# Sangluisme/PSgradientSDF

Hardware: AMD Instinct MI355X
Metric: Gauss-Newton iterations/sec (full PS sweep), 256^3 grid x 50 frames (higher is better)
Workload: dtype f32

## Files before the change

### psgradientsdf_amd/capi.py

```python
from __future__ import annotations

import ctypes as C
import os

import numpy as np

ALBEDO, LIGHT, DIST, POSE, ALL = 1, 2, 4, 8, 15
SH1, SH2, LED = 0, 1, 2
L2, CAUCHY, HUBER, TUKEY, TRUNC_L2 = 0, 1, 2, 3, 4
R_DEPTH, R_NORMAL, R_ALBEDO, R_SHADING, R_RENDERED, R_RESIDUAL, R_VOXEL = 1, 2, 4, 8, 16, 32, 64
R_ALL = 127
_R_PLANES = [("depth", R_DEPTH, 1), ("normal", R_NORMAL, 3), ("albedo", R_ALBEDO, 3), ("shading", R_SHADING, 1),
             ("rendered", R_RENDERED, 3), ("residual", R_RESIDUAL, 3), ("voxel", R_VOXEL, 1)]

_HERE = os.path.dirname(os.path.abspath(__file__))
ENGINE_LIB = os.environ.get("PSGSDF_ENGINE_LIB") or os.path.join(_HERE, "csrc", "libpsgsdf.so")
ENGINE_LIB_DEV = os.path.join(_HERE, "csrc", "libpsgsdf_dev.so")


class GridDesc(C.Structure):
    _fields_ = [("dim", C.c_int32 * 3), ("voxel_size", C.c_float), ("shift", C.c_float * 3), ("truncation", C.c_float)]


class Settings(C.Structure):
# ... 439 lines not shown
    def watch_kernel(self, name):
        self._check(self._fn("watch_kernel")(self.ctx, name.encode() if name else None), "watch_kernel")

    def reset_kernel_times(self):
        self._check(self._fn("reset_kernel_times")(self.ctx), "reset_kernel_times")

    def kernel_times(self):
        cap = 64
        names = (C.c_char_p * cap)(); ms = (C.c_double * cap)(); n = (C.c_int64 * cap)()
        f = getattr(self._lib, self._p + "kernel_times"); f.restype = C.c_int
        k = f(self.ctx, names, ms, n, C.c_int(cap))
        return {names[i].decode(): (ms[i], n[i]) for i in range(k)}

    def debug_dist_system(self, x=None):
        S = self.info().n_band
        diag = np.empty(S, np.float32); rhs = np.empty(S, np.float32)
        y = np.empty(S, np.float32) if x is not None else None
        xa = np.ascontiguousarray(x, np.float32) if x is not None else None
        self._check(self._fn("debug_dist_system")(self.ctx, diag.ctypes.data_as(C.c_void_p), rhs.ctypes.data_as(C.c_void_p),
                                                   xa.ctypes.data_as(C.c_void_p) if x is not None else None,
                                                   y.ctypes.data_as(C.c_void_p) if x is not None else None), "debug_dist_system")
        return diag, rhs, y

    def debug_time_pcg_pass(self, blocks=0, rows=2, ablate=0, reps=50, stamps=False):
        ms = C.c_double(0)
        st = np.zeros((max(blocks, 1), 8), np.int64) if stamps else None
        self._check(self._fn("debug_time_pcg_pass")(self.ctx, C.c_int(blocks), C.c_int(rows), C.c_int(ablate | (1024 if stamps else 0)), C.c_int(reps), C.byref(ms),
                                                     st.ctypes.data_as(C.c_void_p) if stamps else None), "debug_time_pcg_pass")
        return (ms.value, st) if stamps else ms.value

    def debug_time_pcg_solve(self, passes=16, reps=5):
        ms = C.c_double(0); shape = (C.c_int32 * 2)(); st = (C.c_double * 16)()
        self._check(self._fn("debug_time_pcg_solve")(self.ctx, C.c_int(passes), C.c_int(reps), C.byref(ms), shape, st), "debug_time_pcg_solve")
        return ms.value, (shape[0], shape[1]), [x for x in st]

    def debug_sync_stats(self):
        out = (C.c_int64 * 8)()
        self._check(self._fn("debug_sync_stats")(self.ctx, out), "debug_sync_stats")
        return dict(readbacks_checked=out[0], readbacks_late=out[1], persist_fallbacks=out[2] % 1000000, keyframes_compacted=out[2] // 1000000, speculative_starts=out[3] // 1000000, speculative_undos=out[3] % 1000000,
                    cross_rank_ready=out[4] % 10, halo_pushes=out[4] // 10, cross_rank_solves=out[5], cross_rank_mem_kind=out[6], probe_stale=out[7] // 1000000, probe_timeouts=out[7] % 1000000)

    def debug_rare_rows(self):
        r = C.c_int64(); w = C.c_int64()
        self._check(self._fn("debug_rare_rows")(self.ctx, C.byref(r), C.byref(w)), "debug_rare_rows")
        return r.value, w.value

# ... 79 lines not shown
```

### psgradientsdf_amd/csrc/api_debug.hip

```cpp
#include "engine_internal.h"

using namespace psge;

extern "C" {
int psgsdf_set_profiling(psgsdf_ctx* c, int enabled) { if (!c) return PSGSDF_ERR_ARG; c->profiling = enabled != 0; return PSGSDF_OK; }
int psgsdf_reset_kernel_times(psgsdf_ctx* c) { if (!c) return PSGSDF_ERR_ARG; c->ktimes.clear(); c->watch_used = 0; return PSGSDF_OK; }
int psgsdf_watch_kernel(psgsdf_ctx* c, const char* name) {
    if (!c) return PSGSDF_ERR_ARG;
    hipStreamSynchronize(c->stream);
    std::string w = name ? name : ""; int every = 1;
    const size_t sl = w.find('/');
    if (sl != std::string::npos) { every = std::max(1, atoi(w.c_str() + sl + 1)); w.resize(sl); }
    c->watch = w; c->watch_every = every; c->watch_seen = 0; c->watch_used = 0;
    return PSGSDF_OK;
}
int psgsdf_kernel_times(psgsdf_ctx* c, const char** names, double* ms, int64_t* launches, int cap) {
    if (!c) return 0;
    if (c->watch_used) {
        hipStreamSynchronize(c->stream);
        KTime& k = c->ktimes[c->watch];
        for (size_t i = 0; i < c->watch_used; ++i) { float t = 0; if (hipEventElapsedTime(&t, c->watch_pool[i].first, c->watch_pool[i].second) == hipSuccess) { k.ms += t; k.n += 1; } }
        c->watch_used = 0;
    }
    int n = 0;
    for (auto& kv : c->ktimes) { if (n >= cap) break; names[n] = kv.first.c_str(); ms[n] = kv.second.ms; launches[n] = kv.second.n; ++n; }
    return n;
}

int psgsdf_debug_dist_system(psgsdf_ctx* c, float* diag, float* rhs, const float* x, float* y) {
    if (!c || !c->inited) return fail(c, PSGSDF_ERR_STATE, "init first");
    HIPCHK(c, hipSetDevice(c->device));
    SweepArgs a = make_args(c, c->reg_l != 0.f);
    launch_sweep_dist(a, c->stream);
    launch_assemble(a, c->stream);
    const int S = c->band.S;
    if (diag) HIPCHK(c, hipMemcpyAsync(diag, c->band.H, sizeof(float) * S, hipMemcpyDeviceToHost, c->stream));
    if (rhs) HIPCHK(c, hipMemcpyAsync(rhs, c->band.rhs, sizeof(float) * S, hipMemcpyDeviceToHost, c->stream));
    if (x && y) {
        HIPCHK(c, hipMemcpyAsync(c->band.x, x, sizeof(float) * S, hipMemcpyHostToDevice, c->stream));
        launch_matvec(a, c->band.x, c->band.t, c->stream);
        HIPCHK(c, hipMemcpyAsync(y, c->band.t, sizeof(float) * S, hipMemcpyDeviceToHost, c->stream));
    }
    HIPCHK(c, hipStreamSynchronize(c->stream));
    return PSGSDF_OK;
}

int psgsdf_debug_time_pcg_pass(psgsdf_ctx* c, int blocks, int rows, int ablate, int reps, double* avg_ms, long long* stamps) {
    if (!c || !c->inited || !avg_ms) return fail(c, PSGSDF_ERR_STATE, "init first");
    HIPCHK(c, hipSetDevice(c->device));
    SweepArgs a = make_args(c, c->reg_l != 0.f);
    launch_sweep_dist(a, c->stream);
    launch_assemble(a, c->stream);
    int G, rdef; cgf_shape(band_blocks(c), &G, &rdef);
    if (blocks > 0) G = std::min(blocks, kCgfMaxBlocks);
    if (rows <= 0) rows = rdef;
    launch_cgf_init(a, c->pcg_sc, c->pcg_part, G, c->stream);
    hipEvent_t e0, e1; HIPCHK(c, hipEventCreate(&e0)); HIPCHK(c, hipEventCreate(&e1));
    for (int q = 0; q < 3; ++q) launch_cgf_pass(a, c->pcg_sc, c->pcg_part, G, rows, q, 1 << 30, c->mbox_dev, c->stream, ablate | 16);
    HIPCHK(c, hipEventRecord(e0, c->stream));
    for (int q = 0; q < reps; ++q) launch_cgf_pass(a, c->pcg_sc, c->pcg_part, G, rows, 3 + q, 1 << 30, c->mbox_dev, c->stream, ablate | 16);
    HIPCHK(c, hipEventRecord(e1, c->stream));
    HIPCHK(c, hipStreamSynchronize(c->stream));
    float ms = 0; HIPCHK(c, hipEventElapsedTime(&ms, e0, e1));
    hipEventDestroy(e0); hipEventDestroy(e1);
    *avg_ms = (double)ms / reps;
    if (stamps) {
// ... 216 lines not shown
```

### psgradientsdf_amd/csrc/band.hip

```cpp
#include "device_common.h"

namespace psg {


__global__ void __launch_bounds__(kBlock) k_select_vis(const uint64_t* __restrict__ vis_seq, int wpv_seq, uint64_t* __restrict__ vis_key, int KW, const int* __restrict__ frame_idx, int F, long long nvox) {
    for (long long lin = blockIdx.x * (long long)blockDim.x + threadIdx.x; lin < nvox; lin += (long long)gridDim.x * blockDim.x) {
        if (wpv_seq <= 2) {
            const uint64_t s0 = vis_seq[lin * wpv_seq], s1 = wpv_seq > 1 ? vis_seq[lin * wpv_seq + 1] : 0ull;
            for (int w = 0; w < KW; ++w) {
                uint64_t out = 0;
                if (s0 | s1) {
                    const int f1 = min(F, 64 * (w + 1));
                    for (int f = 64 * w; f < f1; ++f) {
                        const int s = frame_idx[f];
                        const uint64_t word = s < 64 ? s0 : s1;
                        if (s >= 0 && s < 64 * wpv_seq && ((word >> (s & 63)) & 1ull)) out |= 1ull << (f & 63);
                    }
                }
                vis_key[lin * KW + w] = out;
            }
            continue;
        }
        for (int w = 0; w < KW; ++w) {
            uint64_t out = 0;
// ... 109 lines not shown
        if (!(q & 1) && r >= 0) fwd |= 1 << (q >> 1);
    }
    b.dirb[j] = fwd;
    int dl[kNQ], far = 0;
    for (int q = 0; q < kNQ; ++q) {
        int o[3]; q_offset(q, o);
        long long ln = lin + o[0] * stride[0] + o[1] * stride[1] + o[2] * stride[2];
        int r = (ln >= 0 && ln < grid.nvox) ? d.row_of[ln] : -1;
        b.col[(size_t)q * b.Spad + j] = r >= 0 ? r : j;
        dl[q] = r >= 0 ? r - j : 0;
        far = max(far, abs(dl[q]));
    }
    for (int w = 0; w < (kNQ - 1) / 2; ++w)
        b.colp[(size_t)w * b.Spad + j] = ((unsigned)dl[2 * w + 1] & 0xffffu) | ((unsigned)dl[2 * w + 2] << 16);
#pragma unroll
    for (int o = 32; o > 0; o >>= 1) far = max(far, __shfl_down(far, o, 64));
    if ((threadIdx.x & 63) == 0 && far > 0) atomicMax(reach, far);
}
void launch_band_fill(const DenseView& d, const GridP& grid, Band b, int* d_reach, hipStream_t s) {
    int g1 = (int)min((grid.nvox + kBlock - 1) / kBlock, (long long)256 * 16);
    hipLaunchKernelGGL(k_band_fill, dim3(g1), dim3(kBlock), 0, s, d, grid, b);
    if (b.S > 0) hipLaunchKernelGGL(k_band_nb, dim3((b.S + kBlock - 1) / kBlock), dim3(kBlock), 0, s, d, grid, b, d_reach);
}
__global__ void __launch_bounds__(kBlock) k_band_scatter(DenseView d, Band b) {
    int j = blockIdx.x * blockDim.x + threadIdx.x;
    if (j >= b.S) return;
    long long lin = b.lin[j];
    d.dist[lin] = b.dist[j];
#pragma unroll
    for (int a = 0; a < 3; ++a) { d.g[a][lin] = b.g[a][j]; d.rho[a][lin] = b.rho[a][j]; }
}
void launch_band_scatter(const DenseView& d, Band b, hipStream_t s) {
    if (b.S > 0) hipLaunchKernelGGL(k_band_scatter, dim3((b.S + kBlock - 1) / kBlock), dim3(kBlock), 0, s, d, b);
}

__global__ void __launch_bounds__(kBlock) k_upsample(DenseView src, DenseView dst, GridP g) {
    const long long nx = 2LL * g.dim[0], ny = 2LL * g.dim[1], nn = 8 * g.nvox;
    const float vs4 = (float)(0.25 * (double)g.vs);
    for (long long ls = blockIdx.x * (long long)blockDim.x + threadIdx.x; ls < nn; ls += (long long)gridDim.x * blockDim.x) {
        long long kz = ls / (nx * ny); long long rest = ls - kz * nx * ny; long long jy = rest / nx; long long ix = rest - jy * nx;
        long long lin = (ix >> 1) + (jy >> 1) * g.dim[0] + (kz >> 1) * (long long)g.dim[0] * g.dim[1];
        float d = src.dist[lin];
        if (d == g.T) {
            dst.dist[ls] = g.T; dst.weight[ls] = 0.f;
#pragma unroll
            for (int a = 0; a < 3; ++a) { dst.g[a][ls] = 0.f; dst.rho[a][ls] = 0.5f; }
// ... 148 lines not shown
```

### psgradientsdf_amd/csrc/device_common.h

```cpp
#pragma once
#include "engine.h"
#include <float.h>

#ifndef PSG_STRICT
#define PSG_STRICT 0
#endif
#if PSG_STRICT & 1
#pragma clang fp contract(off)
#else
#pragma clang fp contract(fast)
#endif

namespace psg {
#if PSG_STRICT & 8
typedef double obs_acc_t;
#else
typedef float obs_acc_t;
#endif

typedef float f2_t __attribute__((ext_vector_type(2)));
__device__ __forceinline__ float dot3(const float* a, const float* b) { return (a[0] * b[0] + a[1] * b[1]) + a[2] * b[2]; }
__device__ __forceinline__ float norm3(const float* a) { return sqrtf(dot3(a, a)); }
__device__ __forceinline__ void normalized3(const float* v, float* o) {
#pragma clang fp contract(off)
// ... 629 lines not shown
    float e = norm3(n) - 1; en = (double)(e * e);
    float l = laplacian(b, j, a.grid.vs_inv); el = (double)(l * l);
}

#define FOR_EACH_VISIBLE_FRAME(b, j, F, f)                                                   \
    for (int _w = 0; _w < (b).KW; ++_w)                                                      \
        for (uint64_t _m = (b).vis[(size_t)_w * (b).Spad + (j)]; _m; _m &= _m - 1)            \
            if (int f = 64 * _w + __builtin_ctzll(_m); f < (F))

struct PiRows { float p00, p02, p11, p12; };
__device__ __forceinline__ PiRows pi_rows(const Cam& cam, const Proj& pr) {
    const float z_inv = pr.z_inv, z_inv_sq = z_inv * z_inv;
    PiRows o; o.p00 = cam.fx * z_inv; o.p02 = -cam.fx * pr.p[0] * z_inv_sq; o.p11 = cam.fy * z_inv; o.p12 = -cam.fy * pr.p[1] * z_inv_sq;
    return o;
}
__device__ __forceinline__ void pi_rows_world(const PiRows& pi, const float* R, float* U, float* V) {
#pragma unroll
    for (int k = 0; k < 3; ++k) { U[k] = pi.p00 * R[k * 3 + 0] + pi.p02 * R[k * 3 + 2]; V[k] = pi.p11 * R[k * 3 + 1] + pi.p12 * R[k * 3 + 2]; }
}
__device__ __forceinline__ int sym4(int a, int b) {
    if (a > b) { int t = a; a = b; b = t; }
    return a * 4 - (a * (a - 1)) / 2 + (b - a);
}

__device__ inline void so3_exp(const float* w, float* R) {
    float theta_sq = dot3(w, w);
    float imag, real;
    if (theta_sq < 1e-10f) {
        float theta_po4 = theta_sq * theta_sq;
        imag = 0.5f - (1.0f / 48.0f) * theta_sq + (1.0f / 3840.0f) * theta_po4;
        real = 1.0f - (1.0f / 8.0f) * theta_sq + (1.0f / 384.0f) * theta_po4;
    } else {
        float theta = sqrtf(theta_sq), half = 0.5f * theta;
        imag = sinf(half) / theta; real = cosf(half);
    }
    float qw = real, qx = imag * w[0], qy = imag * w[1], qz = imag * w[2];
    float tx = 2 * qx, ty = 2 * qy, tz = 2 * qz;
    float twx = tx * qw, twy = ty * qw, twz = tz * qw, txx = tx * qx, txy = ty * qx, txz = tz * qx, tyy = ty * qy, tyz = tz * qy, tzz = tz * qz;
    R[0] = 1 - (tyy + tzz); R[1] = txy - twz; R[2] = txz + twy;
    R[3] = txy + twz; R[4] = 1 - (txx + tzz); R[5] = tyz - twx;
    R[6] = txz - twy; R[7] = tyz + twx; R[8] = 1 - (txx + tyy);
}
__device__ inline void pose_update(FrameP* frames, int f, const float* xi) {
    float R[9], t[3];
    for (int i = 0; i < 9; ++i) R[i] = frames[f].R[i];
    for (int i = 0; i < 3; ++i) t[i] = frames[f].t[i];
// ... 10 lines not shown
```

### psgradientsdf_amd/csrc/dist.hip

```cpp
#include "device_common.h"

#ifndef PSG_DIST_PK
#define PSG_DIST_PK 1
#endif

namespace psg {

__device__ __forceinline__ void normal_jacobian(float vs_inv, const float* grad, const float* direction, float* J) {
    float n_d[3] = {-vs_inv * direction[0], -vs_inv * direction[1], -vs_inv * direction[2]};
    float N_inv = (float)(1.0 / (double)fmaxf(norm3(grad), 0.001f));
    double Nd = (double)N_inv;
    float dN = (float)((Nd * Nd * Nd) * (double)dot3(n_d, grad));
#pragma unroll
    for (int k = 0; k < 3; ++k) J[k] = N_inv * n_d[k] - dN * grad[k];
}

template <int MODEL, int LOSS, int IMG>
__global__ void __launch_bounds__(kBlock, 4) k_sweep_dist(SweepArgs a) {
    constexpr int NB = ModelTraits<MODEL>::NB;
    constexpr bool LED = ModelTraits<MODEL>::LED;
    FrameP* sf = reinterpret_cast<FrameP*>(psg_dyn_smem);
    __shared__ double red[kBlock / 64];
    load_frames(sf, a.frames, a.F);
    const Band& b = a.b;
// ... 215 lines not shown
            float n_d[3] = {-vs_inv * dir[0], -vs_inv * dir[1], -vs_inv * dir[2]};
            float Jr[4];
            Jr[0] = dot3(grad, n_d);
#pragma unroll
            for (int k = 0; k < 3; ++k) Jr[k + 1] = grad[k] * (vs_inv * dir[k]);
            float gnrm = norm3(grad);
            if (gnrm > 0.0f) {
#pragma unroll
                for (int k = 0; k < 4; ++k) Jr[k] /= gnrm;
            }
            float res = gnrm - 1;
            int q = 0;
#pragma unroll
            for (int p = 0; p < 4; ++p) {
#pragma unroll
                for (int k = p; k < 4; ++k) B[q++] += (obs_acc_t)(a.reg_n * (Jr[p] * Jr[k]));
                g[p] += (obs_acc_t)(a.reg_n * (Jr[p] * res));
            }
        }
        if (a.laplacian_reg) {
            float vs2 = vs_inv * vs_inv; float Jl = -6 * vs2; float res = laplacian(b, j, vs_inv);
            B[0] += (obs_acc_t)(a.reg_l * (Jl * Jl)); g[0] += (obs_acc_t)(a.reg_l * (Jl * res));
        }
        int q = 0;
#pragma unroll
        for (int p = 0; p < 4; ++p) {
#pragma unroll
            for (int k = p; k < 4; ++k) { b.blk[(size_t)q * b.Spad + j] = (exists[p] && exists[k]) ? (float)B[q] : 0.f; ++q; }
        }
#pragma unroll
        for (int p = 0; p < 4; ++p) b.blk[(size_t)(10 + p) * b.Spad + j] = exists[p] ? (float)g[p] : 0.f;
    }
    block_part_store(E, PART(a, SC_ENERGY), red, bid);
    block_part_store(nobs, PART(a, SC_NOBS), red, bid);
    if (a.pcg_asm && a.pcg_gran) {
        if (blockIdx.x == 0 && threadIdx.x == 0) { a.pcg_fs[1] = 0.0; a.pcg_fs[2] = 0.0; a.pcg_fs[3] = 0.0; }
        const int gid = blockIdx.x * blockDim.x + threadIdx.x;
        for (int q = gid; q < a.pcg_gran_n; q += gridDim.x * blockDim.x) a.pcg_gran[q] = 0.0;
    }
}
void launch_sweep_dist(const SweepArgs& a, hipStream_t s) {
    if (a.row1 <= a.row0) return;
    dim3 g((a.row1 - a.row0 + kBlock - 1) / kBlock), bl(kBlock);
    PSG_LAUNCH_SWEEP(k_sweep_dist, a, false, g, bl, a.F * sizeof(FrameP), s, a);
}

__device__ __forceinline__ double assemble_row(const SweepArgs& a, int i, double (*acc)[kBlock]) {
    const Band& b = a.b;
    const int tid = threadIdx.x;
    double bb = 0.0;
    int jr[7]; jr[0] = i;
#pragma unroll
    for (int c = 1; c < 7; ++c) { const int ax = (c - 1) >> 1; const bool upper = (c - 1) & 1; jr[c] = b.nb[(size_t)(2 * ax + (upper ? 0 : 1)) * b.Spad + i]; }
    int db[7];
#pragma unroll
    for (int c = 0; c < 7; ++c) db[c] = b.dirb[jr[c] >= 0 ? jr[c] : i];
    bool use[7]; use[0] = true;
#pragma unroll
    for (int c = 1; c < 7; ++c) { const int ax = (c - 1) >> 1; const bool upper = (c - 1) & 1; use[c] = jr[c] >= 0 && !(upper && ((db[c] >> ax) & 1)); }
    float val[7][4], gr[7];
#pragma unroll
    for (int c = 0; c < 7; ++c) {
        const int s = c == 0 ? 0 : ((c - 1) >> 1) + 1;
        const int jrow = use[c] ? jr[c] : i;
        gr[c] = b.blk[(size_t)(10 + s) * b.Spad + jrow];
#pragma unroll
        for (int bq = 0; bq < 4; ++bq) val[c][bq] = b.blk[(size_t)sym4(s, bq) * b.Spad + jrow];
    }
    double rhs = 0.0;
#pragma unroll
    for (int c = 0; c < 7; ++c) {
        if (!use[c]) continue;
        const int ax = c == 0 ? 0 : (c - 1) >> 1; const bool upper = c > 0 && ((c - 1) & 1);
        int coff[3] = {0, 0, 0};
        if (c > 0) coff[ax] = upper ? 1 : -1;
        rhs += (double)gr[c];
#pragma unroll
        for (int bq = 0; bq < 4; ++bq) {
            int o[3] = {coff[0], coff[1], coff[2]};
            if (bq > 0) o[bq - 1] += ((db[c] >> (bq - 1)) & 1) ? 1 : -1;
            if (val[c][bq] != 0.f) acc[q_of(o)][tid] += (double)val[c][bq];
        }
    }
    int extra = 0;
#pragma unroll
    for (int q = 0; q < kNQ; ++q) { float h = (float)acc[q][tid]; b.H[(size_t)q * b.Spad + i] = h; if (q >= kNQCommon && h != 0.f) extra = 1; }
    b.hx[i] = extra;
    b.rhs[i] = (float)rhs;
    if (a.pcg_fuse_init) {
        float dg = (float)acc[0][tid];
        if (a.damping != 0.0f) dg += a.damping * dg;
// ... 32 lines not shown
```

### psgradientsdf_amd/csrc/engine.h

```cpp
#pragma once
#include <hip/hip_runtime.h>
#include <stdint.h>

namespace psg {

constexpr int kBlock = 256;
constexpr int kMaxFramesLds = 640;
constexpr int kNQ = 19;
constexpr int kNQCommon = 13;
constexpr int kMaxBasis = 9;

struct FrameP {
    float R[9];
    float t[3];
    float l[9];
    float pad[3];
};

struct Cam { float fx, fy, cx, cy; int W, H; };

struct GridP {
    int dim[3];
    long long nvox;
    float vs, vs_inv;
// ... 1 lines not shown
    float T;
    int koff;
};

struct Robust { int loss; float lambda, lambda_sq, inv_lambda; };

struct Band {
    int S, Spad, KW;
    int* lin;
    float* dist;
    float* g[3];
    float* rho[3];
    uint64_t* vis;
    int* nb;
    int* dirb;
    float* nbd;
    int* col;
    unsigned* colp;
    int col16;
    int reach;
    float* gfd[3];
    float4* vp[3];
    float* aH; float* ab;
    float* blk;
    float* H;
    int* hx;
    float* rhs; float* x; float* t;
    float4* rec[2];
    int* obs_ptr;
    int* obs_rows;
    int obs_max;
    long long obs_ptr_total;
};

struct Accum {
    double* frame;
    double* part;
    int PB;
    double* fpart;
    int fcap;
    int* fdone;
};
constexpr int kFrameRow = 64;
constexpr int kPcgMaxBlocks = 2048;
constexpr int kCgfMaxBlocks = 768;

enum { SC_ENERGY = 0, SC_NOBS = 1, SC_EN = 2, SC_EL = 3, SC_ACCEPT = 4, SC_AUX0 = 5, SC_AUX1 = 6, SC_AUX2 = 7, SC_COUNT = 8 };
// ... 57 lines not shown
};

constexpr int kXrMaxRanks = 32;
constexpr int kXrPeerTags = 64;
constexpr int kXrRankGran = 0, kXrPtag = 2 * 8 * kXrMaxRanks, kXrAbort = kXrPtag + 2 * 3 * kXrPeerTags, kXrDoubles = kXrAbort + 8;
constexpr int kXrLate = kXrAbort + 1;
constexpr int kXrNonce = kXrAbort + 7;
struct XrArgs {
    int rank, n_ranks;
    double* region[kXrMaxRanks];
    float4* lo_rec[2]; float4* hi_rec[2];
    float4* lo_base[2];
    int give_lo, give_hi;
    int wait_lo, wait_hi;
    int need_lo, need_hi;
    unsigned epoch;
};
struct XfTable {
    int n_ranks, rank, F, spin_max;
    long long pay, flg;
    long long spay, sflg;
    double* region[32];
};
constexpr int kHxWords = 16;
constexpr unsigned kXrEpochMask = 0x3fffu;

constexpr int kTryPackFlags = 2048;
void launch_normals_cache(int W, int H, int r, double fx_inv, double fy_inv, double cx, double cy, double* work , float* out , hipStream_t s);
void launch_try_pack_f32(const float* rgb, unsigned* rgba, size_t npix, size_t stride, float scale, int* fail , hipStream_t s);
void launch_pack_rgb8(const uint8_t* rgb, unsigned* rgba, size_t npix, hipStream_t s);
void launch_select_vis(const uint64_t* vis_seq, int wpv_seq, uint64_t* vis_key, int KW, const int* frame_idx, int F, long long nvox, hipStream_t s);
void launch_band_flags(const float* dist, const uint64_t* vis_key, int KW, float vs, long long nvox, int* flags, hipStream_t s);
void launch_band_scan(int* flags_inout_rowof, long long nvox, int* block_sums, int* d_total, hipStream_t s);
struct DenseView { float* dist; float* g[3]; float* weight; float* rho[3]; uint64_t* vis; int KW; int* row_of; };
void launch_band_fill(const DenseView& d, const GridP& grid, Band b, int* d_reach, hipStream_t s);
void launch_band_scatter(const DenseView& d, Band b, hipStream_t s);
void launch_derive(const SweepArgs& a, int update_grad, hipStream_t s);
constexpr int kObsChunk = 2048;
void launch_obs_count(const Band& b, int F, int row0, int row1, int* counts, hipStream_t s);
void launch_block_work(const Band& b, int row0, int row1, int* work, hipStream_t s);
void launch_obs_fill(const Band& b, int F, int row0, int row1, const int* offsets, hipStream_t s);
void launch_lower_bound(const int* lin, int S, int target, int* out, hipStream_t s);
struct SlotList { int n; int id[8]; };
void launch_sum_parts(const double* part, int PB, int nblk, const SlotList& slots, double* out, unsigned long long key, hipStream_t s, const XfTable* xf = nullptr, long long xf_epoch = 0);
void launch_frame_cols(const double* frame, int F, int col, double* out, unsigned long long key, hipStream_t s);
void launch_zero_f64(double* p, int n, hipStream_t s);
struct CopySegs { int n; unsigned off[16]; unsigned len[16]; unsigned long long key[16]; };
void launch_copy_segs(const double* src, double* dst, const CopySegs& segs, hipStream_t s);
void launch_marker(double* p, double v, hipStream_t s);
void launch_init_albedo(const SweepArgs& a, hipStream_t s);
void launch_led_light_init(const SweepArgs& a, hipStream_t s);
void launch_energy(const SweepArgs& a, hipStream_t s);
void launch_sweep_albedo(const SweepArgs& a, hipStream_t s);
void launch_apply_albedo(const SweepArgs& a, hipStream_t s);
void launch_restore_albedo(const SweepArgs& a, hipStream_t s);
int launch_sweep_light(const SweepArgs& a, hipStream_t s);
int launch_sweep_pose(const SweepArgs& a, hipStream_t s);
void launch_solve_light(const SweepArgs& a, FrameP* frames, float* led_light, double* e_out, unsigned long long e_key, float* undo, hipStream_t s);
// ... 92 lines not shown
```

### psgradientsdf_amd/csrc/engine.hip

```cpp
#include "engine_internal.h"
#include <chrono>
#include <sched.h>

namespace psge {

int wait_mapped(psgsdf_ctx* c, const std::function<bool()>& ready, const char* what) {
    using clk = std::chrono::steady_clock;
    static const double limit_s = [] { const char* e = getenv("PSGSDF_WAIT_TIMEOUT_S"); double v = e ? atof(e) : 0.0; return v > 0.0 ? v : 120.0; }();
    clk::time_point t0{}, next_query{};
    bool timing = false;
    for (unsigned spin = 1;; ++spin) {
        if (ready()) return 0;
        if (spin & 0x3ffu) continue;
        const clk::time_point now = clk::now();
        if (!timing) { timing = true; t0 = now; next_query = now + std::chrono::milliseconds(20); continue; }
        if (now - t0 > std::chrono::milliseconds(2)) sched_yield();
        if (now < next_query) continue;
        next_query = now + std::chrono::milliseconds(20);
        const hipError_t q = hipStreamQuery(c->stream);
        if (q == hipSuccess) return ready() ? 0 : 1;
        if (q != hipErrorNotReady) return fail(c, PSGSDF_ERR_DEVICE, "%s: stream error while waiting: %s", what, hipGetErrorString(q));
        if (std::chrono::duration<double>(now - t0).count() > limit_s)
            return fail(c, PSGSDF_ERR_DEVICE, "%s: nothing published within %.0f s (PSGSDF_WAIT_TIMEOUT_S)", what, limit_s);
    }
// ... 193 lines not shown
    HIPCHK(c, hipMalloc(&d.dist, sizeof(float) * nvox));
    for (int a = 0; a < 3; ++a) { HIPCHK(c, hipMalloc(&d.g[a], sizeof(float) * nvox)); HIPCHK(c, hipMalloc(&d.rho[a], sizeof(float) * nvox)); }
    HIPCHK(c, hipMalloc(&d.weight, sizeof(float) * nvox));
    d.KW = KW;
    if (KW > 0) HIPCHK(c, hipMalloc(&d.vis, sizeof(uint64_t) * nvox * KW));
    if (with_rowof) HIPCHK(c, hipMalloc(&d.row_of, sizeof(int) * nvox));
    return 0;
}

int build_band(psgsdf_ctx* c) {
    if (!c->deferred.empty() || c->pending_fold.n) { int rc = flush(c); if (rc) return rc; }
    if (xr_quiesce(c, 120.0)) return fail(c, PSGSDF_ERR_COMM, "band rebuild: a rank never closed its mappings of this rank's record planes (lost or failed peer?)");
    if (c->n_ranks > 1 && c->comm) { int rc = xr_probe(c); if (rc) return rc; }
    c->persist_off = false;
    const long long nvox = c->grid.nvox;
    const int KW = c->dense.KW;
    if (!c->block_sums) HIPCHK(c, hipMalloc(&c->block_sums, sizeof(int) * ((nvox + 1023) / 1024 + 1)));
    timed(c, "band_flags", [&] { launch_band_flags(c->dense.dist, c->dense.vis, KW, c->grid.vs, nvox, c->dense.row_of, c->stream); });
    timed(c, "band_scan", [&] { launch_band_scan(c->dense.row_of, nvox, c->block_sums, c->d_total, c->stream); });
    int S = 0;
    HIPCHK(c, hipMemcpyAsync(&S, c->d_total, sizeof(int), hipMemcpyDeviceToHost, c->stream));
    HIPCHK(c, hipStreamSynchronize(c->stream));
    const int Spad = ((S + kBlock - 1) / kBlock) * kBlock + kBlock;
    const size_t n4 = 1 + 1 + 3 + 3 + 6 + 6 + kNQ + 12 + 6 + 14 + kNQ + 4 + 9 + 1 + 3;
    const size_t bytes = (n4 * 4 + (size_t)KW * 8) * Spad + 256;
    if (c->band_mem) { hipFree(c->band_mem); c->band_mem = nullptr; }
    if (c->rec_mem) { hipFree(c->rec_mem); c->rec_mem = nullptr; }
    HIPCHK(c, hipMalloc(&c->band_mem, bytes));
    HIPCHK(c, hipMemsetAsync(c->band_mem, 0, bytes, c->stream));
    { int rc = xr_alloc(c, &c->rec_mem, 2 * sizeof(float4) * (size_t)Spad, false); if (rc) return rc; }
    HIPCHK(c, hipMemsetAsync(c->rec_mem, 0, 2 * sizeof(float4) * (size_t)Spad, c->stream));
    c->band_bytes = bytes;
    char* p = (char*)c->band_mem;
    auto take = [&](size_t elems, size_t esz) { void* r = p; p += elems * esz * Spad; return r; };
    Band& b = c->band;
    b.S = S; b.Spad = Spad; b.KW = KW;
    b.vis = (uint64_t*)take(KW, 8);
    b.rec[0] = (float4*)c->rec_mem; b.rec[1] = b.rec[0] + Spad;
    b.lin = (int*)take(1, 4);
    b.dist = (float*)take(1, 4);
    for (int a = 0; a < 3; ++a) b.g[a] = (float*)take(1, 4);
    for (int a = 0; a < 3; ++a) b.rho[a] = (float*)take(1, 4);
    b.nb = (int*)take(6, 4); b.nbd = (float*)take(6, 4); b.col = (int*)take(kNQ, 4); b.colp = (unsigned*)take(9, 4); b.dirb = (int*)take(1, 4);
    for (int a = 0; a < 3; ++a) b.gfd[a] = (float*)take(1, 4);
    for (int a = 0; a < 3; ++a) b.vp[a] = (float4*)take(4, 4);
    b.aH = (float*)take(3, 4); b.ab = (float*)take(3, 4);
    b.blk = (float*)take(14, 4); b.H = (float*)take(kNQ, 4);
    b.hx = (int*)take(1, 4);
    b.rhs = (float*)take(1, 4); b.x = (float*)take(1, 4); b.t = (float*)take(1, 4);
    if ((size_t)(p - (char*)c->band_mem) > bytes) return fail(c, PSGSDF_ERR_DEVICE, "band arena overrun: %zu > %zu bytes", (size_t)(p - (char*)c->band_mem), bytes);
    HIPCHK(c, hipMemsetAsync(c->d_total, 0, sizeof(int), c->stream));
    timed(c, "band_fill", [&] { launch_band_fill(c->dense, c->grid, b, c->d_total, c->stream); });
    {
        int reach = 0;
        HIPCHK(c, hipMemcpyAsync(&reach, c->d_total, sizeof(int), hipMemcpyDeviceToHost, c->stream));
        HIPCHK(c, hipStreamSynchronize(c->stream));
        b.col16 = reach <= 32767; b.reach = reach;
        if (const char* e = getenv("PSGSDF_PCG_COL16")) if (atoi(e) == 0) b.col16 = 0;
    }
    {
        c->row0 = 0; c->row1 = S;
        c->halo = 0; c->need[0] = c->need[1] = 0; c->give[0] = c->give[1] = 0; c->halo_active = false;
        if (c->n_ranks > 1 && !c->comm) return fail(c, PSGSDF_ERR_COMM, "rank %d of %d has no communicator (psgsdf_comm_init)", c->rank, c->n_ranks);
        if (3 * c->n_ranks > kMgScal) return fail(c, PSGSDF_ERR_UNSUPPORTED, "at most %d ranks", kMgScal / 3);
        if (c->n_ranks > 1) {
            const long long plane = (long long)c->grid.dim[0] * c->grid.dim[1];
            int rr[2] = {0, S};
            if (S > 0) {
                launch_lower_bound(b.lin, S, (int)((c->z0 - c->zlo) * plane), c->d_need, c->stream);
                launch_lower_bound(b.lin, S, (int)((c->z1 - c->zlo) * plane), c->d_need + 1, c->stream);
// ... 1 lines not shown
                HIPCHK(c, hipStreamSynchronize(c->stream));
            }
            c->row0 = rr[0]; c->row1 = rr[1];
            c->need[0] = c->row0; c->need[1] = S - c->row1; c->halo = std::max(c->need[0], c->need[1]);
            std::vector<double> info(3 * (size_t)c->n_ranks, 0.0);
            info[3 * c->rank] = c->need[0]; info[3 * c->rank + 1] = c->need[1]; info[3 * c->rank + 2] = c->row1 - c->row0;
            HIPCHK(c, hipMemcpyAsync(c->mg_scal, info.data(), sizeof(double) * info.size(), hipMemcpyHostToDevice, c->stream));
            int rcc = comm_allreduce(c, c->mg_scal, (int)info.size()); if (rcc) return rcc;
            HIPCHK(c, hipMemcpyAsync(info.data(), c->mg_scal, sizeof(double) * info.size(), hipMemcpyDeviceToHost, c->stream));
            HIPCHK(c, hipStreamSynchronize(c->stream));
            const int own = c->row1 - c->row0;
            if (c->rank > 0) c->give[0] = std::min((int)info[3 * (c->rank - 1) + 1], own);
            if (c->rank < c->n_ranks - 1) c->give[1] = std::min((int)info[3 * (c->rank + 1)], own);
            c->S_global = 0;
            for (int r = 0; r < c->n_ranks; ++r) {
                if (info[3 * r] != 0.0 || info[3 * r + 1] != 0.0) c->halo_active = true;
                if (info[3 * r + 2] == 0.0) return fail(c, PSGSDF_ERR_UNSUPPORTED, "rank %d of %d owns no band rows: use fewer ranks", r, c->n_ranks);
                c->S_global += (long long)info[3 * r + 2];
            }
            int hrc = comm_halo(c, b.dirb, 1, 1); if (hrc) return hrc;
            if ((hrc = xr_setup(c, info))) return hrc;
        } else c->S_global = S;
    }
    if (c->areg_mem) { hipFree(c->areg_mem); c->areg_mem = nullptr; c->ar = AlbedoReg{}; }
    if (c->reg_r != 0.f) {
        const size_t planes = 3 + 1 + 9 + 12 + 3 + 8 * 3 + 1;
        HIPCHK(c, hipMalloc(&c->areg_mem, planes * 4 * (size_t)Spad));
        HIPCHK(c, hipMemsetAsync(c->areg_mem, 0, planes * 4 * (size_t)Spad, c->stream));
        char* q = (char*)c->areg_mem;
        auto tk = [&](size_t n) { void* r = q; q += n * 4 * (size_t)Spad; return r; };
        AlbedoReg& ar = c->ar;
        ar.anb = (int*)tk(3); ar.back = (int*)tk(1); ar.anrho = (float*)tk(9); ar.J = (float*)tk(12); ar.res = (float*)tk(3);
        ar.rhs = (float*)tk(3); ar.diag = (float*)tk(3); ar.diag0 = (float*)tk(3); ar.x = (float*)tk(3); ar.r = (float*)tk(3); ar.p = (float*)tk(3); ar.q = (float*)tk(3); ar.t = (float*)tk(3); ar.cgs = (double*)tk(1);
        SweepArgs at{}; at.b = b; at.ar = ar;
        launch_areg_tables(c->dense, c->grid, at, c->stream);
        if (int hrc = comm_halo(c, ar.back, 1, 1)) return hrc;
    }
    {
        const int nch = (c->row1 - c->row0 + kObsChunk - 1) / kObsChunk, F = c->F;
        if (c->obs_mem) { hipFree(c->obs_mem); c->obs_mem = nullptr; }
        b.obs_ptr = nullptr; b.obs_rows = nullptr; b.obs_max = 0; b.obs_ptr_total = 0;
        if (nch > 0 && F > 0) {
            int* d_counts = nullptr;
            HIPCHK(c, hipMalloc(&d_counts, sizeof(int) * (size_t)nch * F));
            launch_obs_count(b, F, c->row0, c->row1, d_counts, c->stream);
            std::vector<int> cnt((size_t)nch * F), off((size_t)nch * F), ptr(F + 1);
// ... 92 lines not shown
```

### psgradientsdf_amd/csrc/loop.hip

```cpp
#include "engine_internal.h"
#include <climits>

namespace psge {

constexpr int kCgfSumsHost = 7;
void cgf_shape(int nblk, int* G, int* rows) {
    nblk = std::max(1, nblk);
    int r = 1, cap = kCgfMaxBlocks;
    if (const char* e = getenv("PSGSDF_PCG_ROWS")) { int v = atoi(e); if (v >= 1 && v <= 2) r = v; }
    if (const char* e = getenv("PSGSDF_PCG_BLOCKS")) { int v = atoi(e); if (v > 0 && v <= kCgfMaxBlocks) cap = v; }
    const int per = (nblk + r - 1) / r;
    const int trips = (per + cap - 1) / cap;
    *G = (per + trips - 1) / trips; *rows = r;
}

bool cgf_solve_shape(psgsdf_ctx* c, int* G, int* rows_per_wg, bool any_ranks) {
    if (!c->pcg_persist || c->persist_off || (c->n_ranks > 1 && !c->xr_ready && !any_ranks) || !c->band.col16 || !c->fuse_pcg_init || c->num_cu <= 0 || band_blocks(c) > kPcgMaxBlocks) return false;
    const int n = c->row1 - c->row0, cap = std::min(c->num_cu, kSolveMaxBlocksHost);
    if (n <= 0) return false;
    int g = std::min(cap, (n + kSolveThreadsHost - 1) / kSolveThreadsHost);
    g = std::max(8, g / 8 * 8);
    if (g > cap) g = cap;
    const int per = ((n + g - 1) / g + 63) / 64 * 64;
    const int r = (per + kSolveThreadsHost - 1) / kSolveThreadsHost;
// ... 297 lines not shown
            }
            else timed(c, "solve_light", [&] { launch_solve_light(a, c->frames, c->led_light, c->frame_e_slot, c->frame_e_key, c->spec_undo ? (float*)c->frames_undo : nullptr, c->stream); });
            if (c->spec_undo) c->spec_light_saved = true;
            c->frame_e_slot = nullptr; c->frame_e_key = 0;
            st->cg_converged = 1; st->applied = 1; st->n_accepted = led ? 1 : c->F;
            if (c->frame_solve == 1 && c->want_counts) { if ((rc = read_frame_solver_stats(c, 0, st))) return rc; }
            break;
        case PSGSDF_POSE:
            if (c->fm_solved) c->fm_solved = false;
            else if (c->frame_solve == 1) {
                if (!frames_eigen_fits(c->set.model, c->F)) return fail(c, PSGSDF_ERR_UNSUPPORTED, "PSGSDF_FRAME_SOLVE=eigen holds at most 2048 unknowns in its one workgroup (%d keyframes)", c->F);
                timed(c, "solve_pose_eigen", [&] { launch_frames_eigen_pose(a, c->frames, c->frame_e_slot, c->frame_e_key, c->fs_stats + 4, c->stream); });
            }
            else timed(c, "solve_pose", [&] { launch_solve_pose(a, c->frames, c->frame_e_slot, c->frame_e_key, c->stream); });
            c->frame_e_slot = nullptr; c->frame_e_key = 0;
            st->cg_converged = 1; st->applied = 1; st->n_accepted = c->F;
            if (c->frame_solve == 1 && c->want_counts) { if ((rc = read_frame_solver_stats(c, 1, st))) return rc; st->n_accepted = st->applied ? c->F : 0; }
            break;
        case PSGSDF_DIST: {
            take_fold(c, a, 0u);
            if (c->fuse_pcg_init && band_blocks(c) <= kPcgMaxBlocks) { a.pcg_fuse_init = 1; a.pcg_init_blocks = band_blocks(c); }
            bool apply_in_solve = false;
            { int Gs, Rs; if (a.pcg_fuse_init && cgf_solve_shape(c, &Gs, &Rs)) { a.pcg_gran = c->pcg_gran; a.pcg_gran_n = 2 * kSolveGranPlanes * kSolveMaxBlocksHost; a.pcg_asm = c->pcg_fuse_asm ? 1 : 0; apply_in_solve = a.pcg_asm && c->pcg_fuse_apply && Gs <= band_blocks(c); } }
            if ((rc = comm_halo(c, c->band.blk, 14, 1))) return rc;
            if (!a.pcg_asm) { timed(c, "assemble", [&] { launch_assemble(a, c->stream); }); a.fold.n = 0; }
            int iters = 0, ok = 1; double err = 0;
            const bool only_on_success = !led && c->set.ref_quirks;
            if (apply_in_solve) a.pcg_apply = only_on_success ? 2 : 1;
            bool tail_ran = false; int tail_rc = 0;
            auto tail = [&](const double* gate) {
                SweepArgs ag = a; ag.fold.n = 0; ag.gate = gate;
                if (!a.pcg_apply) timed(c, "apply_dist", [&] { launch_apply_dist(ag, c->stream); });
                if (int hrc = comm_halo(c, c->band.dist, 1, 1)) tail_rc = hrc;
                SweepArgs a2 = make_args(c, 0); a2.gate = gate;
                timed(c, "derive", [&] { launch_derive(a2, 1, c->stream); });
            };
            if ((rc = pcg_solve(c, a, &iters, &ok, &err, tail, only_on_success, &tail_ran))) return rc;
            if (tail_rc) return tail_rc;
            int apply = 1;
            if (only_on_success && !ok) apply = 0;
            if (apply) {
                if (!tail_ran) { tail(nullptr); if (tail_rc) return tail_rc; }
                const int slots[3] = {SC_ACCEPT, SC_EN, SC_EL}; double s[3];
                if (defer_reg_sums) { if ((rc = read_parts_deferred(c, slots, 3, [c](const double* v) { c->en_sum = v[1]; c->el_sum = v[2]; }))) return rc; }
                else { if ((rc = read_parts(c, slots, 3, s))) return rc; st->n_accepted = (int64_t)s[0]; c->en_sum = s[1]; c->el_sum = s[2]; }
            }
            st->cg_iters = iters; st->cg_converged = ok; st->cg_error = err; st->applied = apply;
// ... 219 lines not shown
```

### psgradientsdf_amd/csrc/pcg.hip

```cpp
#include "device_common.h"

namespace psg {

__device__ __forceinline__ float pcg_threshold(float rhsNorm2) { return fmaxf(FLT_EPSILON * FLT_EPSILON * rhsNorm2, FLT_MIN); }


template <int N> struct PartLoads { double ld[kCgfMaxBlocks / kBlock][N]; };
template <int N>
__device__ __forceinline__ void block_total_issue(double* const* src, int n, PartLoads<N>& pl) {
#pragma unroll
    for (int j = 0; j < kCgfMaxBlocks / kBlock; ++j) {
        const int i = threadIdx.x + j * kBlock;
#pragma unroll
        for (int q = 0; q < N; ++q) pl.ld[j][q] = i < n ? src[q][i] : 0.0;
    }
}
template <int N>
__device__ __forceinline__ void block_total_finish(const PartLoads<N>& pl, double* red , double* out) {
    double v[8];
#pragma unroll
    for (int q = 0; q < 8; ++q) v[q] = 0.0;
#pragma unroll
    for (int q = 0; q < N; ++q) {
        v[q] = pl.ld[0][q];
// ... 243 lines not shown
constexpr int kSolveThreads = 512;
constexpr int kSolveMaxBlocks = 256;
constexpr int kSolveMaxRows = 4;
typedef float v4f_t __attribute__((ext_vector_type(4)));
__device__ __forceinline__ void store16_sc1(float4* p, const float4& v) {
    const v4f_t d = {v.x, v.y, v.z, v.w};
    asm volatile("global_store_dwordx4 %0, %1, off sc1\n\ts_nop 1" :: "v"(p), "v"(d) : "memory");
}
__device__ __forceinline__ void store16_sys(float4* p, const float4& v) {
    const v4f_t d = {v.x, v.y, v.z, v.w};
    asm volatile("global_store_dwordx4 %0, %1, off sc0 sc1\n\ts_nop 1" :: "v"(p), "v"(d) : "memory");
}
__device__ __forceinline__ double gran_tag(double v, unsigned tag) { return __longlong_as_double((long long)(((unsigned long long)__double_as_longlong(v) & ~3ull) | tag)); }
__device__ __forceinline__ unsigned gran_tag_of(double v) { return (unsigned)((unsigned long long)__double_as_longlong(v) & 3ull); }
__device__ __forceinline__ double xr_tag(double v, unsigned tag) { return __longlong_as_double((long long)(((unsigned long long)__double_as_longlong(v) & ~0xffffull) | tag)); }
__device__ __forceinline__ unsigned xr_tag_of(double v) { return (unsigned)((unsigned long long)__double_as_longlong(v) & 0xffffull); }

__device__ __forceinline__ bool ell_valid(const int* o) {
    const int nz = (o[0] != 0) + (o[1] != 0) + (o[2] != 0);
    return nz <= 2 && o[0] >= -1 && o[0] <= 1 && o[1] >= -1 && o[1] <= 1 && o[2] >= -1 && o[2] <= 1;
}
__device__ __forceinline__ void assemble_row_regs(const SweepArgs& a, int i, double (&acc)[kNQ], double& rhs) {
    const Band& b = a.b;
    int jr[7]; jr[0] = i;
#pragma unroll
    for (int c = 1; c < 7; ++c) { const int ax = (c - 1) >> 1; const bool upper = (c - 1) & 1; jr[c] = b.nb[(size_t)(2 * ax + (upper ? 0 : 1)) * b.Spad + i]; }
    int db[7];
#pragma unroll
    for (int c = 0; c < 7; ++c) db[c] = b.dirb[jr[c] >= 0 ? jr[c] : i];
    bool use[7]; use[0] = true;
#pragma unroll
    for (int c = 1; c < 7; ++c) { const int ax = (c - 1) >> 1; const bool upper = (c - 1) & 1; use[c] = jr[c] >= 0 && !(upper && ((db[c] >> ax) & 1)); }
    float val[7][4], gr[7];
#pragma unroll
    for (int c = 0; c < 7; ++c) {
        const int sl = c == 0 ? 0 : ((c - 1) >> 1) + 1;
        const int jrow = use[c] ? jr[c] : i;
        gr[c] = b.blk[(size_t)(10 + sl) * b.Spad + jrow];
#pragma unroll
        for (int bq = 0; bq < 4; ++bq) val[c][bq] = b.blk[(size_t)sym4(sl, bq) * b.Spad + jrow];
    }
#pragma unroll
    for (int q = 0; q < kNQ; ++q) acc[q] = 0.0;
    rhs = 0.0;
#pragma unroll
    for (int c = 0; c < 7; ++c) {
        const int ax = c == 0 ? 0 : (c - 1) >> 1; const bool upper = c > 0 && ((c - 1) & 1);
        int coff[3] = {0, 0, 0};
        if (c > 0) coff[ax] = upper ? 1 : -1;
        rhs += use[c] ? (double)gr[c] : 0.0;
#pragma unroll
        for (int bq = 0; bq < 4; ++bq) {
            const double v = use[c] ? (double)val[c][bq] : 0.0;
            if (bq == 0) { acc[q_of(coff)] += v; continue; }
            const bool fwd = (db[c] >> (bq - 1)) & 1;
            int oP[3] = {coff[0], coff[1], coff[2]}, oM[3] = {coff[0], coff[1], coff[2]};
            oP[bq - 1] += 1; oM[bq - 1] -= 1;
            if (ell_valid(oP)) acc[q_of(oP)] += fwd ? v : 0.0;
            if (ell_valid(oM)) acc[q_of(oM)] += fwd ? 0.0 : v;
        }
    }
}

template <int R, bool ASM, bool MR>
// ... 802 lines not shown
```

Baseline: 2898.

## Pack per-voxel 4x4 blocks as float4 and precompute neighbour contributor table

The distance sweep now stores each voxel's 4x4 normal-equation block as four float4 rows plus one float4 gradient row, replacing 14 scalar planes. A new setup kernel precomputes a packed per-row contributor table (neighbour index, direction bits, use flag), so assembly reads two uint4 instead of gathering nb and dirb indirectly. The intent is fewer, wider memory transactions and less dependent gather latency in the assembly and fused PCG paths. In exchange, the stored block grows from 14 to 20 floats, the halo exchange moves more data, row indices are capped at 28 bits, and the table must stay in sync with band changes.

```diff
diff --git a/psgradientsdf_amd/capi.py b/psgradientsdf_amd/capi.py
--- a/psgradientsdf_amd/capi.py
+++ b/psgradientsdf_amd/capi.py
@@ -485,6 +485,13 @@
                                                    y.ctypes.data_as(C.c_void_p) if x is not None else None), "debug_dist_system")
         return diag, rhs, y
 
+    def debug_assembly_inputs(self):
+        S = self.info().n_band
+        tab = np.empty((8, S), np.uint32); nb = np.empty((6, S), np.int32); dirb = np.empty(S, np.int32); blk = np.empty((5, S, 4), np.float32)
+        self._check(self._fn("debug_assembly_inputs")(self.ctx, tab.ctypes.data_as(C.c_void_p), nb.ctypes.data_as(C.c_void_p), dirb.ctypes.data_as(C.c_void_p),
+                                                       blk.ctypes.data_as(C.c_void_p)), "debug_assembly_inputs")
+        return tab, nb, dirb, blk
+
     def debug_time_pcg_pass(self, blocks=0, rows=2, ablate=0, reps=50, stamps=False):
         ms = C.c_double(0)
         st = np.zeros((max(blocks, 1), 8), np.int64) if stamps else None
diff --git a/psgradientsdf_amd/csrc/api_debug.hip b/psgradientsdf_amd/csrc/api_debug.hip
--- a/psgradientsdf_amd/csrc/api_debug.hip
+++ b/psgradientsdf_amd/csrc/api_debug.hip
@@ -42,6 +42,26 @@
         HIPCHK(c, hipMemcpyAsync(y, c->band.t, sizeof(float) * S, hipMemcpyDeviceToHost, c->stream));
     }
     HIPCHK(c, hipStreamSynchronize(c->stream));
+    return PSGSDF_OK;
+}
+
+int psgsdf_debug_assembly_inputs(psgsdf_ctx* c, uint32_t* ctab, int32_t* nb, int32_t* dirb, float* blk) {
+    if (!c || !c->inited) return fail(c, PSGSDF_ERR_STATE, "init first");
+    HIPCHK(c, hipSetDevice(c->device));
+    const Band& b = c->band;
+    const size_t S = (size_t)b.S, Sp = (size_t)b.Spad;
+    if (blk) { SweepArgs a = make_args(c, c->reg_l != 0.f); launch_sweep_dist(a, c->stream); }
+    std::vector<uint4> t(ctab ? 2 * S : 0);
+    for (int p = 0; p < 2 && ctab; ++p) HIPCHK(c, hipMemcpyAsync(t.data() + p * S, b.ctab + p * Sp, sizeof(uint4) * S, hipMemcpyDeviceToHost, c->stream));
+    for (int p = 0; p < 6 && nb; ++p) HIPCHK(c, hipMemcpyAsync(nb + p * S, b.nb + p * Sp, sizeof(int) * S, hipMemcpyDeviceToHost, c->stream));
+    if (dirb) HIPCHK(c, hipMemcpyAsync(dirb, b.dirb, sizeof(int) * S, hipMemcpyDeviceToHost, c->stream));
+    for (int p = 0; p < 5 && blk; ++p) HIPCHK(c, hipMemcpyAsync(blk + p * 4 * S, b.blk + p * Sp, sizeof(float4) * S, hipMemcpyDeviceToHost, c->stream));
+    HIPCHK(c, hipStreamSynchronize(c->stream));
+    for (size_t i = 0; i < S && ctab; ++i) {
+        const uint4 t0 = t[i], t1 = t[S + i];
+        const uint32_t w[8] = {t0.x, t0.y, t0.z, t0.w, t1.x, t1.y, t1.z, t1.w};
+        for (int k = 0; k < 8; ++k) ctab[(size_t)k * S + i] = w[k];
+    }
     return PSGSDF_OK;
 }
 
diff --git a/psgradientsdf_amd/csrc/band.hip b/psgradientsdf_amd/csrc/band.hip
--- a/psgradientsdf_amd/csrc/band.hip
+++ b/psgradientsdf_amd/csrc/band.hip
@@ -155,6 +155,25 @@
     hipLaunchKernelGGL(k_band_fill, dim3(g1), dim3(kBlock), 0, s, d, grid, b);
     if (b.S > 0) hipLaunchKernelGGL(k_band_nb, dim3((b.S + kBlock - 1) / kBlock), dim3(kBlock), 0, s, d, grid, b, d_reach);
 }
+__global__ void __launch_bounds__(kBlock) k_band_ctab(Band b) {
+    const int i = blockIdx.x * blockDim.x + threadIdx.x;
+    if (i >= b.S) return;
+    unsigned w[7];
+    w[0] = (unsigned)b.dirb[i];
+#pragma unroll
+    for (int c = 1; c < 7; ++c) {
+        const int ax = (c - 1) >> 1; const bool upper = (c - 1) & 1;
+        const int j = b.nb[(size_t)(2 * ax + (upper ? 0 : 1)) * b.Spad + i];
+        const int db = b.dirb[j >= 0 ? j : i];
+        const bool use = j >= 0 && !(upper && ((db >> ax) & 1));
+        w[c] = ((unsigned)(use ? j : i) << 4) | ((unsigned)(db & 7) << 1) | (use ? 1u : 0u);
+    }
+    b.ctab[i] = make_uint4(w[0], w[1], w[2], w[3]);
+    b.ctab[(size_t)b.Spad + i] = make_uint4(w[4], w[5], w[6], 0u);
+}
+void launch_band_ctab(Band b, hipStream_t s) {
+    if (b.S > 0) hipLaunchKernelGGL(k_band_ctab, dim3((b.S + kBlock - 1) / kBlock), dim3(kBlock), 0, s, b);
+}
 __global__ void __launch_bounds__(kBlock) k_band_scatter(DenseView d, Band b) {
     int j = blockIdx.x * blockDim.x + threadIdx.x;
     if (j >= b.S) return;
diff --git a/psgradientsdf_amd/csrc/device_common.h b/psgradientsdf_amd/csrc/device_common.h
--- a/psgradientsdf_amd/csrc/device_common.h
+++ b/psgradientsdf_amd/csrc/device_common.h
@@ -675,6 +675,18 @@
     if (a > b) { int t = a; a = b; b = t; }
     return a * 4 - (a * (a - 1)) / 2 + (b - a);
 }
+__device__ __forceinline__ void ctab_row(const Band& b, int i, int (&jr)[7], int (&db)[7], bool (&use)[7]) {
+    const uint4 t0 = b.ctab[i], t1 = b.ctab[(size_t)b.Spad + i];
+    const unsigned w[7] = {0u, t0.y, t0.z, t0.w, t1.x, t1.y, t1.z};
+    jr[0] = i; db[0] = (int)t0.x; use[0] = true;
+#pragma unroll
+    for (int c = 1; c < 7; ++c) { jr[c] = (int)(w[c] >> 4); db[c] = (int)(w[c] >> 1) & 7; use[c] = (w[c] & 1u) != 0u; }
+}
+__device__ __forceinline__ void blk_contrib(const Band& b, int sl, int jrow, float (&val)[4], float& gr) {
+    const float4 v = b.blk[(size_t)sl * b.Spad + jrow];
+    val[0] = v.x; val[1] = v.y; val[2] = v.z; val[3] = v.w;
+    gr = reinterpret_cast<const float*>(b.blk + (size_t)4 * b.Spad + jrow)[sl];
+}
 
 __device__ inline void so3_exp(const float* w, float* R) {
     float theta_sq = dot3(w, w);
diff --git a/psgradientsdf_amd/csrc/dist.hip b/psgradientsdf_amd/csrc/dist.hip
--- a/psgradientsdf_amd/csrc/dist.hip
+++ b/psgradientsdf_amd/csrc/dist.hip
@@ -261,14 +261,14 @@
             float vs2 = vs_inv * vs_inv; float Jl = -6 * vs2; float res = laplacian(b, j, vs_inv);
             B[0] += (obs_acc_t)(a.reg_l * (Jl * Jl)); g[0] += (obs_acc_t)(a.reg_l * (Jl * res));
         }
-        int q = 0;
 #pragma unroll
         for (int p = 0; p < 4; ++p) {
-#pragma unroll
-            for (int k = p; k < 4; ++k) { b.blk[(size_t)q * b.Spad + j] = (exists[p] && exists[k]) ? (float)B[q] : 0.f; ++q; }
-        }
-#pragma unroll
-        for (int p = 0; p < 4; ++p) b.blk[(size_t)(10 + p) * b.Spad + j] = exists[p] ? (float)g[p] : 0.f;
+            float m[4];
+#pragma unroll
+            for (int k = 0; k < 4; ++k) m[k] = (exists[p] && exists[k]) ? (float)B[sym4(p, k)] : 0.f;
+            b.blk[(size_t)p * b.Spad + j] = make_float4(m[0], m[1], m[2], m[3]);
+        }
+        b.blk[(size_t)4 * b.Spad + j] = make_float4((float)g[0], exists[1] ? (float)g[1] : 0.f, exists[2] ? (float)g[2] : 0.f, exists[3] ? (float)g[3] : 0.f);
     }
     block_part_store(E, PART(a, SC_ENERGY), red, bid);
     block_part_store(nobs, PART(a, SC_NOBS), red, bid);
@@ -288,24 +288,11 @@
     const Band& b = a.b;
     const int tid = threadIdx.x;
     double bb = 0.0;
-    int jr[7]; jr[0] = i;
-#pragma unroll
-    for (int c = 1; c < 7; ++c) { const int ax = (c - 1) >> 1; const bool upper = (c - 1) & 1; jr[c] = b.nb[(size_t)(2 * ax + (upper ? 0 : 1)) * b.Spad + i]; }
-    int db[7];
-#pragma unroll
-    for (int c = 0; c < 7; ++c) db[c] = b.dirb[jr[c] >= 0 ? jr[c] : i];
-    bool use[7]; use[0] = true;
-#pragma unroll
-    for (int c = 1; c < 7; ++c) { const int ax = (c - 1) >> 1; const bool upper = (c - 1) & 1; use[c] = jr[c] >= 0 && !(upper && ((db[c] >> ax) & 1)); }
+    int jr[7], db[7]; bool use[7];
+    ctab_row(b, i, jr, db, use);
     float val[7][4], gr[7];
 #pragma unroll
-    for (int c = 0; c < 7; ++c) {
-        const int s = c == 0 ? 0 : ((c - 1) >> 1) + 1;
-        const int jrow = use[c] ? jr[c] : i;
-        gr[c] = b.blk[(size_t)(10 + s) * b.Spad + jrow];
-#pragma unroll
-        for (int bq = 0; bq < 4; ++bq) val[c][bq] = b.blk[(size_t)sym4(s, bq) * b.Spad + jrow];
-    }
+    for (int c = 0; c < 7; ++c) blk_contrib(b, c == 0 ? 0 : ((c - 1) >> 1) + 1, jr[c], val[c], gr[c]);
     double rhs = 0.0;
 #pragma unroll
     for (int c = 0; c < 7; ++c) {
diff --git a/psgradientsdf_amd/csrc/engine.h b/psgradientsdf_amd/csrc/engine.h
--- a/psgradientsdf_amd/csrc/engine.h
+++ b/psgradientsdf_amd/csrc/engine.h
@@ -47,7 +47,8 @@
     float* gfd[3];
     float4* vp[3];
     float* aH; float* ab;
-    float* blk;
+    float4* blk;
+    uint4* ctab;
     float* H;
     int* hx;
     float* rhs; float* x; float* t;
@@ -151,7 +152,7 @@
     long long spay, sflg;
     double* region[32];
 };
-constexpr int kHxWords = 16;
+constexpr int kHxWords = 20;
 constexpr unsigned kXrEpochMask = 0x3fffu;
 
 constexpr int kTryPackFlags = 2048;
@@ -163,6 +164,7 @@
 void launch_band_scan(int* flags_inout_rowof, long long nvox, int* block_sums, int* d_total, hipStream_t s);
 struct DenseView { float* dist; float* g[3]; float* weight; float* rho[3]; uint64_t* vis; int KW; int* row_of; };
 void launch_band_fill(const DenseView& d, const GridP& grid, Band b, int* d_reach, hipStream_t s);
+void launch_band_ctab(Band b, hipStream_t s);
 void launch_band_scatter(const DenseView& d, Band b, hipStream_t s);
 void launch_derive(const SweepArgs& a, int update_grad, hipStream_t s);
 constexpr int kObsChunk = 2048;
diff --git a/psgradientsdf_amd/csrc/engine.hip b/psgradientsdf_amd/csrc/engine.hip
--- a/psgradientsdf_amd/csrc/engine.hip
+++ b/psgradientsdf_amd/csrc/engine.hip
@@ -239,7 +239,8 @@
     HIPCHK(c, hipMemcpyAsync(&S, c->d_total, sizeof(int), hipMemcpyDeviceToHost, c->stream));
     HIPCHK(c, hipStreamSynchronize(c->stream));
     const int Spad = ((S + kBlock - 1) / kBlock) * kBlock + kBlock;
-    const size_t n4 = 1 + 1 + 3 + 3 + 6 + 6 + kNQ + 12 + 6 + 14 + kNQ + 4 + 9 + 1 + 3;
+    const size_t n4 = 1 + 1 + 3 + 3 + 6 + 6 + kNQ + 12 + 6 + 20 + 8 + kNQ + 4 + 9 + 1 + 3;
+    if (Spad >= (1 << 28)) return fail(c, PSGSDF_ERR_UNSUPPORTED, "band of %d rows: the contributor table holds 28-bit row numbers", S);
     const size_t bytes = (n4 * 4 + (size_t)KW * 8) * Spad + 256;
     if (c->band_mem) { hipFree(c->band_mem); c->band_mem = nullptr; }
     if (c->rec_mem) { hipFree(c->rec_mem); c->rec_mem = nullptr; }
@@ -262,7 +263,7 @@
     for (int a = 0; a < 3; ++a) b.gfd[a] = (float*)take(1, 4);
     for (int a = 0; a < 3; ++a) b.vp[a] = (float4*)take(4, 4);
     b.aH = (float*)take(3, 4); b.ab = (float*)take(3, 4);
-    b.blk = (float*)take(14, 4); b.H = (float*)take(kNQ, 4);
+    b.blk = (float4*)take(5, 16); b.ctab = (uint4*)take(2, 16); b.H = (float*)take(kNQ, 4);
     b.hx = (int*)take(1, 4);
     b.rhs = (float*)take(1, 4); b.x = (float*)take(1, 4); b.t = (float*)take(1, 4);
     if ((size_t)(p - (char*)c->band_mem) > bytes) return fail(c, PSGSDF_ERR_DEVICE, "band arena overrun: %zu > %zu bytes", (size_t)(p - (char*)c->band_mem), bytes);
@@ -310,6 +311,7 @@
             if ((hrc = xr_setup(c, info))) return hrc;
         } else c->S_global = S;
     }
+    launch_band_ctab(b, c->stream);
     if (c->areg_mem) { hipFree(c->areg_mem); c->areg_mem = nullptr; c->ar = AlbedoReg{}; }
     if (c->reg_r != 0.f) {
         const size_t planes = 3 + 1 + 9 + 12 + 3 + 8 * 3 + 1;
diff --git a/psgradientsdf_amd/csrc/loop.hip b/psgradientsdf_amd/csrc/loop.hip
--- a/psgradientsdf_amd/csrc/loop.hip
+++ b/psgradientsdf_amd/csrc/loop.hip
@@ -343,7 +343,7 @@
             if (c->fuse_pcg_init && band_blocks(c) <= kPcgMaxBlocks) { a.pcg_fuse_init = 1; a.pcg_init_blocks = band_blocks(c); }
             bool apply_in_solve = false;
             { int Gs, Rs; if (a.pcg_fuse_init && cgf_solve_shape(c, &Gs, &Rs)) { a.pcg_gran = c->pcg_gran; a.pcg_gran_n = 2 * kSolveGranPlanes * kSolveMaxBlocksHost; a.pcg_asm = c->pcg_fuse_asm ? 1 : 0; apply_in_solve = a.pcg_asm && c->pcg_fuse_apply && Gs <= band_blocks(c); } }
-            if ((rc = comm_halo(c, c->band.blk, 14, 1))) return rc;
+            if ((rc = comm_halo(c, c->band.blk, 5, 4))) return rc;
             if (!a.pcg_asm) { timed(c, "assemble", [&] { launch_assemble(a, c->stream); }); a.fold.n = 0; }
             int iters = 0, ok = 1; double err = 0;
             const bool only_on_success = !led && c->set.ref_quirks;
diff --git a/psgradientsdf_amd/csrc/pcg.hip b/psgradientsdf_amd/csrc/pcg.hip
--- a/psgradientsdf_amd/csrc/pcg.hip
+++ b/psgradientsdf_amd/csrc/pcg.hip
@@ -289,24 +289,11 @@
 }
 __device__ __forceinline__ void assemble_row_regs(const SweepArgs& a, int i, double (&acc)[kNQ], double& rhs) {
     const Band& b = a.b;
-    int jr[7]; jr[0] = i;
-#pragma unroll
-    for (int c = 1; c < 7; ++c) { const int ax = (c - 1) >> 1; const bool upper = (c - 1) & 1; jr[c] = b.nb[(size_t)(2 * ax + (upper ? 0 : 1)) * b.Spad + i]; }
-    int db[7];
-#pragma unroll
-    for (int c = 0; c < 7; ++c) db[c] = b.dirb[jr[c] >= 0 ? jr[c] : i];
-    bool use[7]; use[0] = true;
-#pragma unroll
-    for (int c = 1; c < 7; ++c) { const int ax = (c - 1) >> 1; const bool upper = (c - 1) & 1; use[c] = jr[c] >= 0 && !(upper && ((db[c] >> ax) & 1)); }
+    int jr[7], db[7]; bool use[7];
+    ctab_row(b, i, jr, db, use);
     float val[7][4], gr[7];
 #pragma unroll
-    for (int c = 0; c < 7; ++c) {
-        const int sl = c == 0 ? 0 : ((c - 1) >> 1) + 1;
-        const int jrow = use[c] ? jr[c] : i;
-        gr[c] = b.blk[(size_t)(10 + sl) * b.Spad + jrow];
-#pragma unroll
-        for (int bq = 0; bq < 4; ++bq) val[c][bq] = b.blk[(size_t)sym4(sl, bq) * b.Spad + jrow];
-    }
+    for (int c = 0; c < 7; ++c) blk_contrib(b, c == 0 ? 0 : ((c - 1) >> 1) + 1, jr[c], val[c], gr[c]);
 #pragma unroll
     for (int q = 0; q < kNQ; ++q) acc[q] = 0.0;
     rhs = 0.0;
```

Result: no change. 2903 (median of 4 runs) (+0.2%).
